# eladhoffer/convNet.pytorch

Measured on NVIDIA H100. Metric: ResNet-50 images/sec (training step, synthetic 224x224), higher is better.
Workload: dtype bf16

## Files before the change

### convnet/pytorch_b200/csrc/bn.cu

```cuda
#include "bn_common.cuh"

namespace b200 {

static inline int reduce_blocks(long long M, int C, const RowMap& rm, int resident_per_sm = 6) {
  long long iters = (M + rm.rows_per_iter - 1) / rm.rows_per_iter;
  long long want = (iters + 7) / 8;
  long long cap = 1200000LL / (2 * C);
  if (cap < sm_count()) cap = sm_count();
  if (cap > resident_per_sm * sm_count()) cap = resident_per_sm * sm_count();
  if (want > cap) want = cap;
  if (want < 1) want = 1;
  return (int)want;
}
__device__ __forceinline__ bool accumulate_and_elect(float (&acc)[16], int cv, int rows_per_iter, int C,
                                                     double* accum, unsigned* ticket) {
  __shared__ float red[kBnThreads][17];
  __shared__ bool is_last;
  const int t = threadIdx.x;
#pragma unroll
  for (int i = 0; i < 16; ++i) red[t][i] = acc[i];
  __syncthreads();
  for (int o = t; o < 2 * C; o += kBnThreads) {
    const int stat = o / C;
    const int c = o - stat * C;
// ... 348 lines not shown
    unsigned long long rm = 0;
    bool ok[ROWS];
    if (SRC == 2) rm = mask_rows<ROWS>(amask, r, C >> 3, (int)(col >> 3)) >> (col & 7 & ~(VEC - 1));
#pragma unroll
    for (int u = 0; u < ROWS; ++u) {
      const long long rr = r + (long long)u * rstep;
      ok[u] = rr < row_end;
      if (ok[u]) {
        rd[u] = ldv(dy + rr * C + col, (RawVec<VEC>*)nullptr);
        rz[u] = ldv(z + rr * C + col, (RawVec<VEC>*)nullptr);
        if (SRC == 1) ry[u] = ldv(y + rr * C + col, (RawVec<VEC>*)nullptr);
      }
    }
#pragma unroll
    for (int u = 0; u < ROWS; ++u) {
      if (!ok[u]) continue;
      const long long rr = r + (long long)u * rstep;
      float da[VEC], za[VEC], ya[VEC];
      unpackv(rd[u], da);
      unpackv(rz[u], za);
      if (SRC == 1) unpackv(ry[u], ya);
#pragma unroll
      for (int i = 0; i < VEC; ++i) {
        float g = da[i];
        if (SRC == 2) g = ((rm >> (8 * u + i)) & 1ull) ? g : 0.f;
        else if (act != B200_ACT_NONE && act_mask(SRC == 1 ? ya[i] : fmaf(za[i], A[i], sh[i]), act) == 0.f) g = 0.f;
        da[i] = g;
        za[i] = A[i] * g + B[i] * za[i] + Cc[i];
      }
      storev(dz + rr * C + col, za);
      if (g_out) storev(g_out + rr * C + col, da);
    }
  }
}

static inline double* ws_accum(float* ws) { return reinterpret_cast<double*>(ws); }
static inline unsigned* ws_ticket(float* ws) { return reinterpret_cast<unsigned*>(ws + kReplicas * 2 * kBnMaxC * 2); }

}

using namespace b200;

extern "C" size_t b200_bn_workspace_floats(int C) { (void)C; return (size_t)kWsFloats; }
extern "C" size_t b200_bn_act_mask_bytes(long long M, int C) { return (size_t)((M + 7) / 8 * 8) * (size_t)(C / 8); }

extern "C" int b200_bn_stats(const void* z, long long M, int C, const float* gamma, const float* beta, float eps,
                             float momentum, float* running_mean, float* running_var, long long* nbt, float* mean,
                             float* invstd, float* scale, float* shift, float* workspace, b200_stream_t stream_) {
  int rc = check_c(C, "bn_stats");
  if (rc) return rc;
  B200_REQUIRE(z && mean && invstd && scale && shift && workspace && M > 0, B200_ERR_INVALID, "bn_stats: bad argument");
  B200_REQUIRE((reinterpret_cast<uintptr_t>(workspace) & 7) == 0, B200_ERR_INVALID, "bn_stats: workspace misaligned");
  const RowMap rm = make_rowmap(C);
  b200::launch(bn_stats_kernel, reduce_blocks(M, C, rm), kBnThreads, 0, (cudaStream_t)stream_,
      (const __nv_bfloat16*)z, M, C, rm.cv, rm.rows_per_iter, gamma, beta, eps, momentum, running_mean, running_var,
      nbt, mean, invstd, scale, shift, ws_accum(workspace), ws_ticket(workspace));
  B200_CHECK_LAUNCH("bn_stats_kernel");
  return B200_OK;
}

extern "C" int b200_bn_finalize(long long M, int C, const float* gamma, const float* beta, float eps, float momentum,
                                float* running_mean, float* running_var, long long* nbt, float* mean, float* invstd,
                                float* scale, float* shift, float* workspace, b200_stream_t stream_) {
  int rc = check_c(C, "bn_finalize");
  if (rc) return rc;
  B200_REQUIRE(mean && invstd && scale && shift && workspace && M > 0, B200_ERR_INVALID, "bn_finalize: bad argument");
// ... 47 lines not shown
extern "C" int b200_bn_bwd_reduce(const void* dy, const void* y, const uint8_t* act_mask, const void* z, long long M,
                                  int C, int act,
                                  const float* mean, const float* invstd, const float* gamma, const float* beta,
                                  float* sums, float* dgamma_acc, float* dbeta_acc, float* workspace,
                                  b200_stream_t stream_) {
  int rc = check_c(C, "bn_bwd_reduce");
  if (rc) return rc;
  B200_REQUIRE(dy && z && mean && invstd && sums && workspace && M > 0, B200_ERR_INVALID, "bn_bwd_reduce: bad argument");
  const int src = (act == B200_ACT_NONE) ? 0 : (act_mask != nullptr ? 2 : (y != nullptr ? 1 : 0));
#define B200_RED_ARGS(VEC)                                                                                     \
  (const __nv_bfloat16*)dy, (const __nv_bfloat16*)y, act_mask, (const __nv_bfloat16*)z, M, C, rm.cv,           \
      rm.rows_per_iter, act, mean, invstd, gamma, beta, partial
#define B200_LAUNCH_RED(VEC, ROWS, MINB)                                                                       \
  do {                                                                                                         \
    const RowMap rm = make_rowmap_v<VEC>(C);                                                                   \
    blocks = partial_blocks(M, rm, MINB);                                                                      \
    if (src == 2)                                                                                              \
      b200::launch(bn_bwd_reduce_kernel<VEC, ROWS, MINB, 2>, blocks, kBnThreads, 0, stream, B200_RED_ARGS(VEC));         \
    else if (src == 1)                                                                                         \
      b200::launch(bn_bwd_reduce_kernel<VEC, ROWS, MINB, 1>, blocks, kBnThreads, 0, stream, B200_RED_ARGS(VEC));         \
    else                                                                                                       \
      b200::launch(bn_bwd_reduce_kernel<VEC, ROWS, MINB, 0>, blocks, kBnThreads, 0, stream, B200_RED_ARGS(VEC));         \
  } while (0)
  cudaStream_t stream = (cudaStream_t)stream_;
  float* partial = workspace + kAccumFloats;
  int blocks = 0;
  if (C > 1024)
    B200_LAUNCH_RED(8, 2, 3);
  else
    B200_LAUNCH_RED(4, 4, 4);
#undef B200_LAUNCH_RED
#undef B200_RED_ARGS
  B200_CHECK_LAUNCH("bn_bwd_reduce_kernel");
  b200::launch(bn_bwd_reduce_final_kernel, (2 * C + 3) / 4, kBnThreads, 0, stream, partial, blocks, C, sums, dgamma_acc,
                                                                           dbeta_acc);
  B200_CHECK_LAUNCH("bn_bwd_reduce_final_kernel");
  return B200_OK;
}

extern "C" int b200_bn_bwd_dx(const void* dy, const void* y, const uint8_t* act_mask, const void* z, long long M, int C,
                              int act,
                              const float* mean, const float* invstd, const float* gamma, const float* beta,
                              const float* sums, void* dz, void* g_out, b200_stream_t stream_) {
  int rc = check_c(C, "bn_bwd_dx");
  if (rc) return rc;
  B200_REQUIRE(dy && z && mean && invstd && sums && dz && M > 0, B200_ERR_INVALID, "bn_bwd_dx: bad argument");
  const int src = (act == B200_ACT_NONE) ? 0 : (act_mask != nullptr ? 2 : (y != nullptr ? 1 : 0));
#define B200_DX_ARGS(VEC)                                                                                    \
  (const __nv_bfloat16*)dy, (const __nv_bfloat16*)y, act_mask, (const __nv_bfloat16*)z, M, C, rm.cv,         \
      rm.rows_per_iter, act, mean, invstd, gamma, beta, sums, (__nv_bfloat16*)dz, (__nv_bfloat16*)g_out
#define B200_LAUNCH_DX(VEC, ROWS, MINB)                                                                      \
  do {                                                                                                       \
    const RowMap rm = make_rowmap_v<VEC>(C);                                                                 \
    const int blocks = stream_blocks(M, rm);                                                                 \
    if (src == 2)                                                                                            \
      b200::launch(bn_bwd_dx_kernel<VEC, ROWS, MINB, 2>, blocks, kBnThreads, 0, (cudaStream_t)stream_, B200_DX_ARGS(VEC)); \
    else if (src == 1)                                                                                       \
      b200::launch(bn_bwd_dx_kernel<VEC, ROWS, MINB, 1>, blocks, kBnThreads, 0, (cudaStream_t)stream_, B200_DX_ARGS(VEC)); \
    else                                                                                                     \
      b200::launch(bn_bwd_dx_kernel<VEC, ROWS, MINB, 0>, blocks, kBnThreads, 0, (cudaStream_t)stream_, B200_DX_ARGS(VEC)); \
  } while (0)
  if (C > 1024)
    B200_LAUNCH_DX(8, 2, 3);
  else
    B200_LAUNCH_DX(4, 4, 4);
#undef B200_LAUNCH_DX
#undef B200_DX_ARGS
  B200_CHECK_LAUNCH("bn_bwd_dx_kernel");
  return B200_OK;
}
// ... 1 lines not shown
```

### convnet/pytorch_b200/csrc/bn_common.cuh

```cuda
#pragma once
#include "common.cuh"
#include "host.h"

namespace b200 {

constexpr int kBnThreads = 256;
constexpr int kBnMaxC = 2048;
constexpr int kBnMaxBlocks = 1184;
constexpr int kAccumFloats = kReplicas * 2 * kBnMaxC * 2 + 64;
constexpr int kMaxPartialBlocks = 6 * 148;
constexpr int kWsFloats = kAccumFloats + kMaxPartialBlocks * 2 * kBnMaxC;

struct RowMap {
  int cv, rows_per_iter;
};
static inline RowMap make_rowmap(int C) {
  RowMap m;
  m.cv = C / 8;
  m.rows_per_iter = kBnThreads / m.cv;
  return m;
}
static inline int partial_blocks(long long M, const RowMap& rm, int resident_per_sm) {
  long long iters = (M + rm.rows_per_iter - 1) / rm.rows_per_iter;
  long long want = (iters + 3) / 4;
// ... 73 lines not shown
__device__ __forceinline__ RawVec<8> ldv(const __nv_bfloat16* p, RawVec<8>*) {
  RawVec<8> r;
  r.u = ld_stream(p);
  return r;
}
__device__ __forceinline__ void unpackv(const RawVec<4>& r, float (&f)[4]) {
  const float2 a = unpack_bf16x2(r.u.x), b = unpack_bf16x2(r.u.y);
  f[0] = a.x; f[1] = a.y; f[2] = b.x; f[3] = b.y;
}
__device__ __forceinline__ void unpackv(const RawVec<8>& r, float (&f)[8]) { unpack8(r.u, f); }
__device__ __forceinline__ void storev(__nv_bfloat16* p, const float (&f)[4]) {
  uint2 u;
  u.x = pack_bf16x2(f[0], f[1]); u.y = pack_bf16x2(f[2], f[3]);
  *reinterpret_cast<uint2*>(p) = u;
}
__device__ __forceinline__ void storev(__nv_bfloat16* p, const float (&f)[8]) { store8(p, f); }
template <int VEC>
__device__ __forceinline__ void loadfv(const float* p, float (&f)[VEC]) {
#pragma unroll
  for (int i = 0; i < VEC; i += 4) {
    const float4 a = __ldg(reinterpret_cast<const float4*>(p + i));
    f[i] = a.x; f[i + 1] = a.y; f[i + 2] = a.z; f[i + 3] = a.w;
  }
}

template <int VEC>
static inline RowMap make_rowmap_v(int C) {
  RowMap m;
  m.cv = C / VEC;
  m.rows_per_iter = kBnThreads / m.cv;
  return m;
}

static int check_c(int C, const char* who) {
  B200_REQUIRE(C > 0 && C % 8 == 0 && C <= kBnMaxC, B200_ERR_UNSUPPORTED,
               "%s: C=%d must be a multiple of 8 and <= %d", who, C, kBnMaxC);
  return B200_OK;
}

}
```

### convnet/pytorch_b200/engine.py

```python
import torch
import torch.nn as nn

from . import ops
from .lib import B200Error, ACT_NONE, ACT_RELU, ACT_RELU6

_ALIGN = 64
FOLD_BN_EVAL = True


def _round_up(n, m):
    return (n + m - 1) // m * m


class _Slot(object):
    __slots__ = ('name', 'param', 'kind', 'offset', 'numel', 'alloc', 'shape', 'group', 'module')


class Arena(object):

    def __init__(self, model, device):
        self.device = device
        self.convs = []
        self.version = 0
        self.grads_zero = False
# ... 369 lines not shown
                            m.num_batches_tracked, u.mean, u.invstd, u.scale, u.shift, self._ws)
        elif training:
            ops.bn_stats(u.z, bn.gamma, bn.beta, m.eps, m.momentum, m.running_mean, m.running_var,
                         m.num_batches_tracked, u.mean, u.invstd, u.scale, u.shift, self._ws)
        else:
            self._eval_coeffs(bn, u.scale, u.shift)
        bias = getattr(u.conv, 'bias32', None) if u.conv is not None else None
        if bias is not None:
            if training:
                if m.momentum is None:
                    m.running_mean.add_(bias / m.num_batches_tracked.to(torch.float32))
                else:
                    m.running_mean.add_(bias, alpha=float(m.momentum))
            else:
                u.shift.add_(u.scale * bias)

    def _stats_only(self, x, conv, bn, training):
        if not training and FOLD_BN_EVAL and not self._want_tape:
            return self._unit_fwd_folded(x, conv, bn, ACT_NONE)
        N, H, W, _ = x.shape
        u = _Unit()
        u.conv, u.bn, u.act, u.x = conv, bn, ACT_NONE, x
        u.desc = conv.desc(N, H, W)
        u.w = conv.kernel_weights()
        self._conv_and_coeffs(u, x, u.w, training)
        u.y = None
        return u

    def _sync_bn_sums(self, sums):
        import torch.distributed as dist
        dist.all_reduce(sums, group=self.sync_bn_group)
        sums.mul_(1.0 / self.sync_bn_world)

    def _bn_bwd(self, u, dy, y_mask, act, want_g=False):
        bn = u.bn
        mask = getattr(u, 'mask', None) if y_mask is not None else None
        ops.bn_bwd_reduce(dy, y_mask, u.z, act, u.mean, u.invstd, bn.gamma, bn.beta, u.sums, bn.dgamma, bn.dbeta,
                          self._ws, act_mask=mask)
        if self.sync_bn_world > 1:
            self._sync_bn_sums(u.sums)
        g = torch.empty_like(dy) if want_g else None
        if bn.l1:
            dz = ops.bn_l1_bwd_dx(dy, y_mask, u.z, act, u.mean, u.invstd, u.sign_sum, bn.gamma, bn.beta, u.sums,
                                  g_out=g, act_mask=mask)
        else:
            dz = ops.bn_bwd_dx(dy, y_mask, u.z, act, u.mean, u.invstd, bn.gamma, bn.beta, u.sums, g_out=g,
                               act_mask=mask)
        return dz, g

    def _wgrad_async(self, fn, *operands):
        if self._wg_stream is None:
            fn()
            return
        ev = torch.cuda.Event()
        ev.record()
        self._wg_stream.wait_event(ev)
        with torch.cuda.stream(self._wg_stream):
            fn()
        self._wg_keep.append(operands)

    def _wgrad_join(self):
        if self._wg_stream is not None and self._wg_keep:
            torch.cuda.current_stream().wait_stream(self._wg_stream)
            self._wg_keep = []

    def _buckets_begin(self):
        self._bucket_hi = self.arena.group_end[0] if self.grad_bucket_hook is not None else None

    def _bucket_point(self, lo, force=False):
# ... 279 lines not shown
            else:
                dws = torch.zeros((K, 9, 16), device=self.device, dtype=torch.float32)
                ops.conv_wgrad(u.x, dz, u.desc, dws)
                self.stem_g32.view(K, 9, Cin).add_(dws[:, :, :Cin])
        self._wgrad_async(stem_wgrad, u.x, dz)

    def _block_fwd(self, spec, x, training):
        convs, bns = spec['convs'], spec['bns']
        units = []
        h = x
        for i in range(len(convs) - 1):
            u = self._unit_fwd(h, convs[i], bns[i], ACT_RELU, training, True)
            units.append(u)
            h = u.y
        down, se_tape = None, None
        if spec.get('se') is not None:
            r = x
            if spec['down'] is not None:
                down = self._unit_fwd(x, spec['down'][0], spec['down'][1], ACT_NONE, training, True)
                r = down.y
            r, se_tape = spec['se'].fwd(r)
            last = self._unit_fwd(h, convs[-1], bns[-1], ACT_RELU, training, True, residual=r)
        elif spec['down'] is not None:
            down = self._stats_only(x, spec['down'][0], spec['down'][1], training)
            last = self._unit_fwd(h, convs[-1], bns[-1], ACT_RELU, training, True, other=down)
        else:
            last = self._unit_fwd(h, convs[-1], bns[-1], ACT_RELU, training, True, residual=x)
        units.append(last)
        return last.y, {'units': units, 'down': down, 'se': se_tape}

    def _block_bwd(self, spec, saved, dy):
        units, down = saved['units'], saved['down']
        last = units[-1]
        dz, g = self._bn_bwd(last, dy, last.y, ACT_RELU, want_g=True)
        if saved.get('se') is not None:
            g = spec['se'].bwd(self, saved['se'], g)
        if down is not None:
            dzd, _ = self._bn_bwd(down, g, None, ACT_NONE)
            skip = self._conv_bwd(down, dzd)
        else:
            skip = g
        d = self._conv_bwd(last, dz)
        for u in reversed(units[1:-1]):
            dz, _ = self._bn_bwd(u, d, None, ACT_RELU)
            d = self._conv_bwd(u, dz)
        u = units[0]
        dz, _ = self._bn_bwd(u, d, None, ACT_RELU)
        return self._conv_bwd(u, dz, residual=skip)

    def run_forward(self, x, training, want_tape, mix=None, aug=None):
        self._want_tape = want_tape
        if training:
            self.arena.version += 1
        h, stem = self._stem_fwd(x, training, mix, aug)
        saved = []
        for spec in self.blocks:
            h, s = self._block_fwd(spec, h, training)
            saved.append(s if want_tape else None)
        out, head = self._head_fwd(h, training, want_tape)
        tape = {'stem': stem, 'blocks': saved, 'head': head} if want_tape else None
        return out, tape

    def run_backward(self, tape, dlogits, dl_bf16=None):
        self._transpose_weights()
        self._buckets_begin()
        d = self._head_bwd(tape['head'], dlogits, dl_bf16)
        for spec, saved in zip(reversed(self.blocks), reversed(tape['blocks'])):
            d = self._block_bwd(spec, saved, d)
            convs = spec['convs'] + ([spec['down'][0]] if spec['down'] is not None else [])
            self._bucket_point(self._spec_lo(convs))
        self._stem_bwd(tape['stem'], d)
        self._wgrad_join()
        self._buckets_end()


class MobileNetRuntime(Runtime):

    def _build(self):
        m, a = self.model, self.arena
        f = m.features
        conv0 = f.conv0[0]
# ... 178 lines not shown
```

### convnet/pytorch_b200/lib.py

```python
import ctypes
import os
import threading

_HERE = os.path.dirname(os.path.abspath(__file__))
LIB_PATH = os.environ.get("B200_LIB_PATH") or os.path.join(_HERE, "libb200conv.so")

ACT_NONE, ACT_RELU, ACT_RELU6 = 0, 1, 2
MIX_NONE, MIX_MIXUP, MIX_CUTMIX = 0, 1, 2


class B200Error(RuntimeError):
    pass


class ConvDesc(ctypes.Structure):
    _fields_ = [(n, ctypes.c_int) for n in
                ("N", "H", "W", "C", "K", "R", "S", "stride", "pad_h", "pad_w", "P", "Q",
                 "x_pixel_stride", "x_row_stride", "x_image_stride", "window")]


class Epilogue(ctypes.Structure):
    _fields_ = [("bias", ctypes.c_void_p), ("residual", ctypes.c_void_p),
                ("act", ctypes.c_int), ("out_fp32", ctypes.c_int), ("bn_stats_workspace", ctypes.c_void_p)]


_vp, _i, _ll, _f, _sz = ctypes.c_void_p, ctypes.c_int, ctypes.c_longlong, ctypes.c_float, ctypes.c_size_t
_dp = ctypes.POINTER(ConvDesc)
_ep = ctypes.POINTER(Epilogue)

SIGNATURES = {
    "b200_conv_fprop": [_dp, _vp, _vp, _vp, _ep, _vp],
    "b200_conv_dgrad": [_dp, _vp, _vp, _vp, _vp, _vp],
    "b200_conv_wgrad": [_dp, _vp, _vp, _vp, _vp, _sz, _vp],
    "b200_conv_wgrad_workspace_bytes": [],
    "b200_dwconv_fprop": [_dp, _vp, _vp, _vp, _vp],
    "b200_dwconv_dgrad": [_dp, _vp, _vp, _vp, _vp],
    "b200_dwconv_wgrad": [_dp, _vp, _vp, _vp, _vp, _sz, _vp],
    "b200_bn_workspace_floats": [_i],
    "b200_bn_act_mask_bytes": [_ll, _i],
    "b200_bn_stats": [_vp, _ll, _i, _vp, _vp, _f, _f, _vp, _vp, _vp, _vp, _vp, _vp, _vp, _vp, _vp],
    "b200_bn_finalize": [_ll, _i, _vp, _vp, _f, _f, _vp, _vp, _vp, _vp, _vp, _vp, _vp, _vp, _vp],
    "b200_bn_eval_coeffs": [_i, _vp, _vp, _vp, _vp, _f, _vp, _vp, _vp],
    "b200_bn_apply": [_vp, _ll, _i, _vp, _vp, _vp, _vp, _vp, _vp, _i, _vp, _vp, _vp],
    "b200_bn_bwd_reduce": [_vp, _vp, _vp, _vp, _ll, _i, _i, _vp, _vp, _vp, _vp, _vp, _vp, _vp, _vp, _vp],
    "b200_bn_bwd_dx": [_vp, _vp, _vp, _vp, _ll, _i, _i, _vp, _vp, _vp, _vp, _vp, _vp, _vp, _vp],
    "b200_bn_l1_stats": [_vp, _ll, _i, _vp, _vp, _f, _f, _vp, _vp, _vp, _vp, _vp, _vp, _vp, _vp, _vp],
    "b200_bn_l1_eval_coeffs": [_i, _vp, _vp, _vp, _vp, _vp, _vp, _vp],
    "b200_bn_l1_bwd_dx": [_vp, _vp, _vp, _vp, _ll, _i, _i, _vp, _vp, _vp, _vp, _vp, _vp, _vp, _vp, _vp],
    "b200_maxpool3x3s2_fwd": [_vp, _i, _i, _i, _i, _vp, _vp, _vp],
    "b200_maxpool3x3s2_bwd": [_vp, _vp, _i, _i, _i, _i, _vp, _vp],
    "b200_bn_apply_maxpool3x3s2": [_vp, _i, _i, _i, _i, _vp, _vp, _i, _vp, _vp, _vp],
    "b200_avgpool_fwd": [_vp, _i, _i, _i, _vp, _vp],
    "b200_avgpool_bwd": [_vp, _i, _i, _i, _vp, _vp],
    "b200_input_prep": [_vp, _i, _i, _i, _i, _i, _i, _vp, _vp],
    "b200_input_prep_u8": [_vp, _i, _i, _i, _i, _i, _i, ctypes.POINTER(ctypes.c_float), ctypes.POINTER(ctypes.c_float),
                           _vp, _vp],
    "b200_input_prep_mix": [_vp, _i, _i, _i, _i, _i, _i, _vp, _vp, _i, _vp, _vp],
    "b200_input_prep_u8_mix": [_vp, _i, _i, _i, _i, _i, _i, ctypes.POINTER(ctypes.c_float),
                               ctypes.POINTER(ctypes.c_float), _vp, _vp, _i, _vp, _vp],
    "b200_input_prep_u8_aug": [_vp, _i, _i, _i, _i, _i, _i, _i, _vp, _vp, _i, _vp, _vp],
    "b200_input_prep_u8_rrc": [_vp, _ll, _vp, _vp, _i, _i, _i, _i, _i, _i, _i, _vp, _vp, _vp],
    "b200_weight_transpose": [_vp, _vp, _i, _i, _i, _vp],
    "b200_weight_transpose_batched": [_vp, _vp, _vp, _i, _i, _vp],
    "b200_stem_weight_to_s2d": [_vp, _i, _i, _i, _vp, _vp],
    "b200_stem_wgrad_from_s2d": [_vp, _i, _i, _i, _vp, _vp],
    "b200_cast_f32_to_bf16": [_vp, _vp, _ll, _vp],
    "b200_group_weight_pack": [_vp, _i, _i, _i, _i, _i, _i, _vp, _vp],
    "b200_group_wgrad_unpack": [_vp, _i, _i, _i, _i, _i, _vp, _vp],
    "b200_se_pool": [_vp, _i, _i, _i, _vp, _vp],
    "b200_se_scale_fwd": [_vp, _vp, _i, _i, _i, _vp, _vp],
    "b200_se_bwd_reduce": [_vp, _vp, _vp, _i, _i, _i, _vp, _vp],
    "b200_se_bwd_dx": [_vp, _vp, _vp, _i, _i, _i, _vp, _vp],
    "b200_act_bwd": [_vp, _vp, _ll, _i, _vp, _vp],
    "b200_softmax_ce": [_vp, _vp, _i, _i, _i, _f, _f, _vp, _vp, _vp, _vp, _vp],
    "b200_softmax_ce_mix": [_vp, _vp, _vp, _vp, _i, _i, _i, _f, _vp, _vp, _vp, _vp, _vp],
    "b200_colsum_bf16": [_vp, _i, _i, _vp, _vp],
    "b200_fused_sgd": [_vp, _vp, _vp, _vp, _ll, _ll, _f, _f, _f, _f, _f, _vp, _i, _i, _vp],
    "b200_sumsq": [_vp, _ll, _vp, _vp, _vp],
# ... 50 lines not shown
```

### convnet/pytorch_b200/ops.py

```python
import ctypes

import torch

from . import lib as _l
from .lib import ACT_NONE, ACT_RELU, ACT_RELU6, ConvDesc, Epilogue

bf16 = torch.bfloat16


def _stream():
    return torch.cuda.current_stream().cuda_stream


_TIMING = None


class _T(object):
    __slots__ = ('name', 'flops', 'nbytes', 'e0')

    def __init__(self, name, flops=0, nbytes=0):
        self.name, self.flops, self.nbytes = name, flops, nbytes

    def __enter__(self):
        if _TIMING is not None:
# ... 208 lines not shown
                 "b200_bn_bwd_reduce")


def bn_bwd_dx(dy, y, z, act, mean, invstd, gamma, beta, sums, dz=None, g_out=None, act_mask=None):
    C = z.shape[-1]
    M = z.numel() // C
    if dz is None:
        dz = torch.empty_like(z)
    with _T('bn_bwd_dx', 0, 2 * z.numel() * (3 + (y is not None and act_mask is None) + (g_out is not None))):
        _l.check(_l.load().b200_bn_bwd_dx(dy.data_ptr(), _l.ptr(y), _l.ptr(act_mask), z.data_ptr(), M, C, int(act),
                                          mean.data_ptr(),
                                          invstd.data_ptr(), _l.ptr(gamma), _l.ptr(beta), sums.data_ptr(),
                                          dz.data_ptr(), _l.ptr(g_out), _stream()), "b200_bn_bwd_dx")
    return dz


def bn_l1_stats(z, gamma, beta, eps, momentum, running_mean, running_var, mean, invstd, sign_sum, scale, shift,
                workspace):
    C = z.shape[-1]
    M = z.numel() // C
    _chk(z, bf16, "z")
    with _T('bn_l1_stats', 0, 2 * 2 * z.numel()):
        _l.check(_l.load().b200_bn_l1_stats(z.data_ptr(), M, C, _l.ptr(gamma), _l.ptr(beta), float(eps),
                                            float(momentum), _l.ptr(running_mean), _l.ptr(running_var),
                                            mean.data_ptr(), invstd.data_ptr(), sign_sum.data_ptr(), scale.data_ptr(),
                                            shift.data_ptr(), workspace.data_ptr(), _stream()), "b200_bn_l1_stats")


def bn_l1_eval_coeffs(gamma, beta, running_mean, running_var, scale, shift):
    C = running_mean.numel()
    _l.check(_l.load().b200_bn_l1_eval_coeffs(C, _l.ptr(gamma), _l.ptr(beta), running_mean.data_ptr(),
                                              running_var.data_ptr(), scale.data_ptr(), shift.data_ptr(), _stream()),
             "b200_bn_l1_eval_coeffs")


def bn_l1_bwd_dx(dy, y, z, act, mean, invstd, sign_sum, gamma, beta, sums, dz=None, g_out=None, act_mask=None):
    C = z.shape[-1]
    M = z.numel() // C
    _chk(dy, bf16, "dy"); _chk(y, bf16, "y"); _chk(z, bf16, "z"); _chk(act_mask, torch.uint8, "act_mask")
    if dz is None:
        dz = torch.empty_like(z)
    with _T('bn_l1_bwd_dx', 0, 2 * z.numel() * (3 + (y is not None and act_mask is None) + (g_out is not None))):
        _l.check(_l.load().b200_bn_l1_bwd_dx(dy.data_ptr(), _l.ptr(y), _l.ptr(act_mask), z.data_ptr(), M, C, int(act),
                                             mean.data_ptr(), invstd.data_ptr(), sign_sum.data_ptr(), _l.ptr(gamma),
                                             _l.ptr(beta), sums.data_ptr(), dz.data_ptr(), _l.ptr(g_out), _stream()),
                 "b200_bn_l1_bwd_dx")
    return dz


def _out(out, shape, dtype, device, name):
    if out is None:
        return torch.empty(shape, device=device, dtype=dtype)
    _chk(out, dtype, name)
    if tuple(out.shape) != tuple(shape):
        raise _l.B200Error("%s has shape %s, expected %s" % (name, tuple(out.shape), tuple(shape)))
    return out


def maxpool_fwd(x, want_argmax=True, out=None, argmax_out=None):
    N, H, W, C = x.shape
    OH, OW = (H - 1) // 2 + 1, (W - 1) // 2 + 1
    y = _out(out, (N, OH, OW, C), bf16, x.device, "out")
    am = _out(argmax_out, (N, OH, OW, C), torch.uint8, x.device, "argmax_out") if want_argmax else None
    with _T('maxpool_fwd', 0, 2 * x.numel() + 3 * y.numel()):
        _l.check(_l.load().b200_maxpool3x3s2_fwd(x.data_ptr(), N, H, W, C, y.data_ptr(), _l.ptr(am), _stream()),
                 "b200_maxpool3x3s2_fwd")
# ... 375 lines not shown
```

### include/b200conv.h

```cpp
#ifndef B200CONV_H_
#define B200CONV_H_

#include <stddef.h>
#include <stdint.h>

#ifdef __cplusplus
extern "C" {
#endif

typedef void* b200_stream_t;

#define B200_OK 0
#define B200_ERR_INVALID (-1)
#define B200_ERR_UNSUPPORTED (-2)
#define B200_ERR_CUDA (-3)

#define B200_ACT_NONE 0
#define B200_ACT_RELU 1
#define B200_ACT_RELU6 2

typedef struct {
  int N, H, W, C;
  int K, R, S;
  int stride;
// ... 19 lines not shown
                    const b200_epilogue* ep, b200_stream_t stream);
int b200_conv_dgrad(const b200_conv_desc* d, const void* dy, const void* wt, void* dx,
                    const void* residual, b200_stream_t stream);
size_t b200_conv_wgrad_workspace_bytes(void);
int b200_conv_wgrad(const b200_conv_desc* d, const void* x, const void* dy, float* dw,
                    void* workspace, size_t workspace_bytes, b200_stream_t stream);

int b200_dwconv_fprop(const b200_conv_desc* d, const void* x, const void* w, void* y, b200_stream_t stream);
int b200_dwconv_dgrad(const b200_conv_desc* d, const void* dy, const void* w, void* dx, b200_stream_t stream);
int b200_dwconv_wgrad(const b200_conv_desc* d, const void* x, const void* dy, float* dw,
                      float* workspace, size_t workspace_bytes, b200_stream_t stream);

size_t b200_bn_workspace_floats(int C);
int b200_bn_stats(const void* z, long long M, int C, const float* gamma, const float* beta,
                  float eps, float momentum, float* running_mean, float* running_var,
                  long long* num_batches_tracked, float* mean, float* invstd, float* scale, float* shift,
                  float* workspace, b200_stream_t stream);
int b200_bn_finalize(long long M, int C, const float* gamma, const float* beta, float eps, float momentum,
                     float* running_mean, float* running_var, long long* num_batches_tracked, float* mean,
                     float* invstd, float* scale, float* shift, float* workspace, b200_stream_t stream);
int b200_bn_eval_coeffs(int C, const float* gamma, const float* beta, const float* running_mean,
                        const float* running_var, float eps, float* scale, float* shift, b200_stream_t stream);
size_t b200_bn_act_mask_bytes(long long M, int C);
int b200_bn_apply(const void* z, long long M, int C, const float* scale, const float* shift,
                  const void* residual, const void* z2, const float* scale2, const float* shift2,
                  int act, void* y, uint8_t* act_mask, b200_stream_t stream);
int b200_bn_bwd_reduce(const void* dy, const void* y, const uint8_t* act_mask, const void* z, long long M, int C, int act,
                       const float* mean, const float* invstd, const float* gamma, const float* beta,
                       float* sums, float* dgamma_acc, float* dbeta_acc, float* workspace, b200_stream_t stream);
int b200_bn_bwd_dx(const void* dy, const void* y, const uint8_t* act_mask, const void* z, long long M, int C, int act,
                   const float* mean, const float* invstd, const float* gamma, const float* beta,
                   const float* sums, void* dz, void* g_out, b200_stream_t stream);

int b200_bn_l1_stats(const void* z, long long M, int C, const float* gamma, const float* beta, float eps,
                     float momentum, float* running_mean, float* running_var, float* mean, float* invstd,
                     float* sign_sum, float* scale, float* shift, float* workspace, b200_stream_t stream);
int b200_bn_l1_eval_coeffs(int C, const float* gamma, const float* beta, const float* running_mean,
                           const float* running_var, float* scale, float* shift, b200_stream_t stream);
int b200_bn_l1_bwd_dx(const void* dy, const void* y, const uint8_t* act_mask, const void* z, long long M, int C,
                      int act, const float* mean, const float* invstd, const float* sign_sum, const float* gamma,
                      const float* beta, const float* sums, void* dz, void* g_out, b200_stream_t stream);

int b200_maxpool3x3s2_fwd(const void* x, int N, int H, int W, int C, void* y, uint8_t* argmax, b200_stream_t stream);
int b200_maxpool3x3s2_bwd(const void* dy, const uint8_t* argmax, int N, int H, int W, int C, void* dx, b200_stream_t stream);
int b200_bn_apply_maxpool3x3s2(const void* z, int N, int H, int W, int C, const float* scale, const float* shift,
                               int act, void* y, uint8_t* argmax, b200_stream_t stream);
int b200_avgpool_fwd(const void* x, int N, int HW, int C, void* y, b200_stream_t stream);
int b200_avgpool_bwd(const void* dy, int N, int HW, int C, void* dx, b200_stream_t stream);

int b200_input_prep(const float* x_nchw, int N, int C, int H, int W, int Cpad, int mode, void* out, b200_stream_t stream);
int b200_input_prep_u8(const uint8_t* x_nhwc, int N, int C, int H, int W, int Cpad, int mode, const float* scale_host,
                       const float* bias_host, void* out, b200_stream_t stream);
#define B200_MIX_NONE 0
#define B200_MIX_MIXUP 1
#define B200_MIX_CUTMIX 2
typedef struct {
  float lam;
  int r0, r1, c0, c1;
} b200_mix_params;
int b200_input_prep_mix(const float* x_nchw, int N, int C, int H, int W, int Cpad, int mode, const long long* perm,
                        const b200_mix_params* params, int kind, void* out, b200_stream_t stream);
int b200_input_prep_u8_mix(const uint8_t* x_nhwc, int N, int C, int H, int W, int Cpad, int mode, const float* scale_host,
                           const float* bias_host, const long long* perm, const b200_mix_params* params, int kind,
                           void* out, b200_stream_t stream);
int b200_input_prep_u8_aug(const uint8_t* x_nhwc, int N, int D, int C, int H, int W, int Cpad, int pad, const float* lut,
                           const int16_t* params, int holes, void* out, b200_stream_t stream);
// ... 42 lines not shown
```

Measured before the change: 6590.

## Fuse last-BN and downsample-BN backward into joint reduce and dx kernels

In downsample bottleneck blocks without SE, the backward pass for the final BN and the downsample BN now runs through joint kernels. These read dy, the ReLU mask and both pre-BN activations once and produce both units' gradient statistics and both dz tensors. The intermediate gradient g is no longer written and re-read, and two reduce/dx kernel pairs become one pair. The cost is more registers per thread, and the two partial buffers now share one workspace, which limits how many blocks the reduce can use.

```diff
diff --git a/convnet/pytorch_b200/csrc/bn.cu b/convnet/pytorch_b200/csrc/bn.cu
--- a/convnet/pytorch_b200/csrc/bn.cu
+++ b/convnet/pytorch_b200/csrc/bn.cu
@@ -404,6 +404,14 @@
       if (g_out) storev(g_out + rr * C + col, da);
     }
   }
+}
+
+int launch_bn_bwd_reduce_final(const float* partial, int nblocks, int C, float* sums, float* dgamma_acc,
+                               float* dbeta_acc, cudaStream_t stream) {
+  b200::launch(bn_bwd_reduce_final_kernel, (2 * C + 3) / 4, kBnThreads, 0, stream, partial, nblocks, C, sums, dgamma_acc,
+               dbeta_acc);
+  B200_CHECK_LAUNCH("bn_bwd_reduce_final_kernel");
+  return B200_OK;
 }
 
 static inline double* ws_accum(float* ws) { return reinterpret_cast<double*>(ws); }
@@ -517,10 +525,7 @@
 #undef B200_LAUNCH_RED
 #undef B200_RED_ARGS
   B200_CHECK_LAUNCH("bn_bwd_reduce_kernel");
-  b200::launch(bn_bwd_reduce_final_kernel, (2 * C + 3) / 4, kBnThreads, 0, stream, partial, blocks, C, sums, dgamma_acc,
-                                                                           dbeta_acc);
-  B200_CHECK_LAUNCH("bn_bwd_reduce_final_kernel");
-  return B200_OK;
+  return launch_bn_bwd_reduce_final(partial, blocks, C, sums, dgamma_acc, dbeta_acc, stream);
 }
 
 extern "C" int b200_bn_bwd_dx(const void* dy, const void* y, const uint8_t* act_mask, const void* z, long long M, int C,
diff --git a/convnet/pytorch_b200/csrc/bn_common.cuh b/convnet/pytorch_b200/csrc/bn_common.cuh
--- a/convnet/pytorch_b200/csrc/bn_common.cuh
+++ b/convnet/pytorch_b200/csrc/bn_common.cuh
@@ -129,6 +129,9 @@
   return m;
 }
 
+int launch_bn_bwd_reduce_final(const float* partial, int nblocks, int C, float* sums, float* dgamma_acc,
+                               float* dbeta_acc, cudaStream_t stream);
+
 static int check_c(int C, const char* who) {
   B200_REQUIRE(C > 0 && C % 8 == 0 && C <= kBnMaxC, B200_ERR_UNSUPPORTED,
                "%s: C=%d must be a multiple of 8 and <= %d", who, C, kBnMaxC);
diff --git a/convnet/pytorch_b200/csrc/bn_join.cu b/convnet/pytorch_b200/csrc/bn_join.cu
--- /dev/null
+++ b/convnet/pytorch_b200/csrc/bn_join.cu
@@ -0,0 +1,221 @@
+#include "bn_common.cuh"
+
+namespace b200 {
+
+template <int VEC, int ROWS, int LB>
+__global__ void __launch_bounds__(kBnThreads, LB) bn_join_bwd_reduce_kernel(
+    const __nv_bfloat16* __restrict__ dy, const uint8_t* __restrict__ amask, const __nv_bfloat16* __restrict__ za,
+    const __nv_bfloat16* __restrict__ zb, long long M, int C, int cv, int rows_per_iter,
+    const float* __restrict__ mean_a, const float* __restrict__ invstd_a, const float* __restrict__ mean_b,
+    const float* __restrict__ invstd_b, float* __restrict__ partial_a, float* __restrict__ partial_b) {
+  const int t = threadIdx.x;
+  const bool active = t < rows_per_iter * cv;
+  const int r0 = t / cv, v = t - r0 * cv;
+  const long long rows_per_block = ((M + gridDim.x - 1) / gridDim.x + 7) & ~7LL;
+  const long long row_begin = blockIdx.x * rows_per_block;
+  const long long row_end = min(M, row_begin + rows_per_block);
+  float acc[3 * VEC];
+#pragma unroll
+  for (int i = 0; i < 3 * VEC; ++i) acc[i] = 0.f;
+  if (active) {
+    float mua[VEC], mub[VEC];
+    loadfv<VEC>(mean_a + v * VEC, mua);
+    loadfv<VEC>(mean_b + v * VEC, mub);
+    const long long col = (long long)v * VEC;
+    for (long long r = row_begin + (long long)r0 * ROWS; r < row_end; r += (long long)ROWS * rows_per_iter) {
+      RawVec<VEC> rd[ROWS], rza[ROWS], rzb[ROWS];
+      bool ok[ROWS];
+      const unsigned long long rm = mask_rows<ROWS>(amask, r, C >> 3, (int)(col >> 3)) >> (col & 7 & ~(VEC - 1));
+#pragma unroll
+      for (int u = 0; u < ROWS; ++u) {
+        const long long rr = r + u;
+        ok[u] = rr < row_end;
+        if (ok[u]) {
+          rd[u] = ldv(dy + rr * C + col, (RawVec<VEC>*)nullptr);
+          rza[u] = ldv(za + rr * C + col, (RawVec<VEC>*)nullptr);
+          rzb[u] = ldv(zb + rr * C + col, (RawVec<VEC>*)nullptr);
+        }
+      }
+#pragma unroll
+      for (int u = 0; u < ROWS; ++u) {
+        if (!ok[u]) continue;
+        float da[VEC], fa[VEC], fb[VEC];
+        unpackv(rd[u], da);
+        unpackv(rza[u], fa);
+        unpackv(rzb[u], fb);
+#pragma unroll
+        for (int i = 0; i < VEC; ++i) {
+          const float g = ((rm >> (8 * u + i)) & 1ull) ? da[i] : 0.f;
+          acc[i] = fmaf(g, fa[i] - mua[i], acc[i]);
+          acc[VEC + i] += g;
+          acc[2 * VEC + i] = fmaf(g, fb[i] - mub[i], acc[2 * VEC + i]);
+        }
+      }
+    }
+    float isa[VEC], isb[VEC];
+    loadfv<VEC>(invstd_a + v * VEC, isa);
+    loadfv<VEC>(invstd_b + v * VEC, isb);
+#pragma unroll
+    for (int i = 0; i < VEC; ++i) {
+      acc[i] *= isa[i];
+      acc[2 * VEC + i] *= isb[i];
+    }
+  }
+  __shared__ float red[kBnThreads][3 * VEC + 1];
+#pragma unroll
+  for (int i = 0; i < 3 * VEC; ++i) red[t][i] = acc[i];
+  __syncthreads();
+  float* dst_a = partial_a + (size_t)blockIdx.x * 2 * C;
+  float* dst_b = partial_b + (size_t)blockIdx.x * 2 * C;
+  for (int o = t; o < 2 * C; o += kBnThreads) {
+    const int stat = o / C;
+    const int c = o - stat * C;
+    const int vv = c / VEC, e = c - vv * VEC;
+    float sa = 0.f, sb = 0.f;
+    for (int r = 0; r < rows_per_iter; ++r) {
+      sa += red[r * cv + vv][stat * VEC + e];
+      sb += red[r * cv + vv][(2 - stat) * VEC + e];
+    }
+    dst_a[o] = sa;
+    dst_b[o] = sb;
+  }
+}
+
+template <int VEC, int ROWS, int LB>
+__global__ void __launch_bounds__(kBnThreads, LB) bn_join_bwd_dx_kernel(
+    const __nv_bfloat16* __restrict__ dy, const uint8_t* __restrict__ amask, const __nv_bfloat16* __restrict__ za,
+    const __nv_bfloat16* __restrict__ zb, long long M, int C, int cv, int rows_per_iter,
+    const float* __restrict__ mean_a, const float* __restrict__ invstd_a, const float* __restrict__ gamma_a,
+    const float* __restrict__ sums_a, const float* __restrict__ mean_b, const float* __restrict__ invstd_b,
+    const float* __restrict__ gamma_b, const float* __restrict__ sums_b, __nv_bfloat16* __restrict__ dza,
+    __nv_bfloat16* __restrict__ dzb) {
+  const int t = threadIdx.x;
+  if (t >= rows_per_iter * cv) return;
+  const int r0 = t / cv, v = t - r0 * cv;
+  const long long rows_per_block = ((M + gridDim.x - 1) / gridDim.x + 7) & ~7LL;
+  const long long row_begin = blockIdx.x * rows_per_block;
+  const long long row_end = min(M, row_begin + rows_per_block);
+  float Aa[VEC], Ba[VEC], Ca[VEC], Ab[VEC], Bb[VEC], Cb[VEC];
+  {
+    const float invM = 1.f / (float)M;
+    const float* mean[2] = {mean_a, mean_b};
+    const float* invstd[2] = {invstd_a, invstd_b};
+    const float* gamma[2] = {gamma_a, gamma_b};
+    const float* sums[2] = {sums_a, sums_b};
+#pragma unroll
+    for (int k = 0; k < 2; ++k) {
+      float mu[VEC], is[VEC], dg[VEC], dbt[VEC], A[VEC];
+      loadfv<VEC>(mean[k] + v * VEC, mu);
+      loadfv<VEC>(invstd[k] + v * VEC, is);
+      if (gamma[k]) loadfv<VEC>(gamma[k] + v * VEC, A);
+      loadfv<VEC>(sums[k] + v * VEC, dg);
+      loadfv<VEC>(sums[k] + C + v * VEC, dbt);
+#pragma unroll
+      for (int i = 0; i < VEC; ++i) {
+        const float gm = gamma[k] ? A[i] : 1.f;
+        const float a = gm * is[i];
+        const float b = -gm * is[i] * is[i] * dg[i] * invM;
+        const float cc = -a * dbt[i] * invM - b * mu[i];
+        if (k == 0) { Aa[i] = a; Ba[i] = b; Ca[i] = cc; } else { Ab[i] = a; Bb[i] = b; Cb[i] = cc; }
+      }
+    }
+  }
+  const long long col = (long long)v * VEC;
+  for (long long r = row_begin + (long long)r0 * ROWS; r < row_end; r += (long long)ROWS * rows_per_iter) {
+    RawVec<VEC> rd[ROWS], rza[ROWS], rzb[ROWS];
+    bool ok[ROWS];
+    const unsigned long long rm = mask_rows<ROWS>(amask, r, C >> 3, (int)(col >> 3)) >> (col & 7 & ~(VEC - 1));
+#pragma unroll
+    for (int u = 0; u < ROWS; ++u) {
+      const long long rr = r + u;
+      ok[u] = rr < row_end;
+      if (ok[u]) {
+        rd[u] = ldv(dy + rr * C + col, (RawVec<VEC>*)nullptr);
+        rza[u] = ldv(za + rr * C + col, (RawVec<VEC>*)nullptr);
+        rzb[u] = ldv(zb + rr * C + col, (RawVec<VEC>*)nullptr);
+      }
+    }
+#pragma unroll
+    for (int u = 0; u < ROWS; ++u) {
+      if (!ok[u]) continue;
+      const long long rr = r + u;
+      float da[VEC], fa[VEC], fb[VEC];
+      unpackv(rd[u], da);
+      unpackv(rza[u], fa);
+      unpackv(rzb[u], fb);
+#pragma unroll
+      for (int i = 0; i < VEC; ++i) {
+        const float g = ((rm >> (8 * u + i)) & 1ull) ? da[i] : 0.f;
+        fa[i] = Aa[i] * g + Ba[i] * fa[i] + Ca[i];
+        fb[i] = Ab[i] * g + Bb[i] * fb[i] + Cb[i];
+      }
+      storev(dza + rr * C + col, fa);
+      storev(dzb + rr * C + col, fb);
+    }
+  }
+}
+
+}
+
+using namespace b200;
+
+extern "C" int b200_bn_join_bwd_reduce(const void* dy, const uint8_t* act_mask, const void* z_a, const void* z_b,
+                                       long long M, int C, const float* mean_a, const float* invstd_a,
+                                       const float* mean_b, const float* invstd_b, float* sums_a, float* sums_b,
+                                       float* dgamma_a, float* dbeta_a, float* dgamma_b, float* dbeta_b,
+                                       float* workspace, b200_stream_t stream_) {
+  int rc = check_c(C, "bn_join_bwd_reduce");
+  if (rc) return rc;
+  B200_REQUIRE(dy && act_mask && z_a && z_b && mean_a && invstd_a && mean_b && invstd_b && sums_a && sums_b &&
+                   workspace && M > 0, B200_ERR_INVALID, "bn_join_bwd_reduce: bad argument");
+  cudaStream_t stream = (cudaStream_t)stream_;
+  float* partial_a = workspace + kAccumFloats;
+  int blocks = 0;
+  float* partial_b = nullptr;
+#define B200_LAUNCH_JRED(VEC, ROWS, MINB, LB)                                                                    \
+  do {                                                                                                           \
+    const RowMap rm = make_rowmap_v<VEC>(C);                                                                     \
+    blocks = partial_blocks(M, rm, MINB);                                                                        \
+    partial_b = partial_a + (size_t)blocks * 2 * C;                                                              \
+    B200_REQUIRE((size_t)blocks * 4 * C <= (size_t)kMaxPartialBlocks * 2 * kBnMaxC, B200_ERR_UNSUPPORTED,         \
+                 "bn_join_bwd_reduce: %d partial rows of two units exceed the workspace (C=%d)", blocks, C);      \
+    b200::launch(bn_join_bwd_reduce_kernel<VEC, ROWS, LB>, blocks, kBnThreads, 0, stream, (const __nv_bfloat16*)dy, \
+                 act_mask, (const __nv_bfloat16*)z_a, (const __nv_bfloat16*)z_b, M, C, rm.cv, rm.rows_per_iter,      \
+                 mean_a, invstd_a, mean_b, invstd_b, partial_a, partial_b);                                      \
+  } while (0)
+  if (C > 1024)
+    B200_LAUNCH_JRED(8, 2, 3, 2);
+  else
+    B200_LAUNCH_JRED(4, 4, 4, 3);
+#undef B200_LAUNCH_JRED
+  B200_CHECK_LAUNCH("bn_join_bwd_reduce_kernel");
+  rc = launch_bn_bwd_reduce_final(partial_a, blocks, C, sums_a, dgamma_a, dbeta_a, stream);
+  if (rc) return rc;
+  return launch_bn_bwd_reduce_final(partial_b, blocks, C, sums_b, dgamma_b, dbeta_b, stream);
+}
+
+extern "C" int b200_bn_join_bwd_dx(const void* dy, const uint8_t* act_mask, const void* z_a, const void* z_b,
+                                   long long M, int C, const float* mean_a, const float* invstd_a,
+                                   const float* gamma_a, const float* sums_a, const float* mean_b,
+                                   const float* invstd_b, const float* gamma_b, const float* sums_b, void* dz_a,
+                                   void* dz_b, b200_stream_t stream_) {
+  int rc = check_c(C, "bn_join_bwd_dx");
+  if (rc) return rc;
+  B200_REQUIRE(dy && act_mask && z_a && z_b && mean_a && invstd_a && sums_a && mean_b && invstd_b && sums_b && dz_a &&
+                   dz_b && M > 0, B200_ERR_INVALID, "bn_join_bwd_dx: bad argument");
+#define B200_LAUNCH_JDX(VEC, ROWS, LB)                                                                           \
+  do {                                                                                                           \
+    const RowMap rm = make_rowmap_v<VEC>(C);                                                                     \
+    b200::launch(bn_join_bwd_dx_kernel<VEC, ROWS, LB>, stream_blocks(M, rm), kBnThreads, 0, (cudaStream_t)stream_, \
+                 (const __nv_bfloat16*)dy, act_mask, (const __nv_bfloat16*)z_a, (const __nv_bfloat16*)z_b, M, C,     \
+                 rm.cv, rm.rows_per_iter, mean_a, invstd_a, gamma_a, sums_a, mean_b, invstd_b, gamma_b, sums_b,    \
+                 (__nv_bfloat16*)dz_a, (__nv_bfloat16*)dz_b);                                                      \
+  } while (0)
+  if (C > 1024)
+    B200_LAUNCH_JDX(8, 2, 2);
+  else
+    B200_LAUNCH_JDX(4, 4, 3);
+#undef B200_LAUNCH_JDX
+  B200_CHECK_LAUNCH("bn_join_bwd_dx_kernel");
+  return B200_OK;
+}
diff --git a/convnet/pytorch_b200/engine.py b/convnet/pytorch_b200/engine.py
--- a/convnet/pytorch_b200/engine.py
+++ b/convnet/pytorch_b200/engine.py
@@ -425,9 +425,9 @@
         dist.all_reduce(sums, group=self.sync_bn_group)
         sums.mul_(1.0 / self.sync_bn_world)
 
-    def _bn_bwd(self, u, dy, y_mask, act, want_g=False):
+    def _bn_bwd(self, u, dy, y_mask, act, want_g=False, act_mask=None):
         bn = u.bn
-        mask = getattr(u, 'mask', None) if y_mask is not None else None
+        mask = act_mask if act_mask is not None else (getattr(u, 'mask', None) if y_mask is not None else None)
         ops.bn_bwd_reduce(dy, y_mask, u.z, act, u.mean, u.invstd, bn.gamma, bn.beta, u.sums, bn.dgamma, bn.dbeta,
                           self._ws, act_mask=mask)
         if self.sync_bn_world > 1:
@@ -773,21 +773,44 @@
     def _block_bwd(self, spec, saved, dy):
         units, down = saved['units'], saved['down']
         last = units[-1]
-        dz, g = self._bn_bwd(last, dy, last.y, ACT_RELU, want_g=True)
-        if saved.get('se') is not None:
+        se = saved.get('se') is not None
+        ds_from_mask = down is not None and not se
+        if ds_from_mask and not last.bn.l1 and not down.bn.l1:
+            dz, dzd = self._bn_join_bwd(last, down, dy)
+            skip = self._conv_bwd(down, dzd)
+            d = self._conv_bwd(last, dz)
+            return self._block_bwd_rest(units, d, skip)
+        dz, g = self._bn_bwd(last, dy, last.y, ACT_RELU, want_g=not ds_from_mask)
+        if se:
             g = spec['se'].bwd(self, saved['se'], g)
-        if down is not None:
+        if ds_from_mask:
+            dzd, _ = self._bn_bwd(down, dy, last.y, ACT_RELU, act_mask=last.mask)
+            skip = self._conv_bwd(down, dzd)
+        elif down is not None:
             dzd, _ = self._bn_bwd(down, g, None, ACT_NONE)
             skip = self._conv_bwd(down, dzd)
         else:
             skip = g
         d = self._conv_bwd(last, dz)
+        return self._block_bwd_rest(units, d, skip)
+
+    def _block_bwd_rest(self, units, d, skip):
         for u in reversed(units[1:-1]):
             dz, _ = self._bn_bwd(u, d, None, ACT_RELU)
             d = self._conv_bwd(u, dz)
         u = units[0]
         dz, _ = self._bn_bwd(u, d, None, ACT_RELU)
         return self._conv_bwd(u, dz, residual=skip)
+
+    def _bn_join_bwd(self, last, down, dy):
+        a, b = last.bn, down.bn
+        ops.bn_join_bwd_reduce(dy, last.mask, last.z, down.z, last.mean, last.invstd, down.mean, down.invstd,
+                               last.sums, down.sums, a.dgamma, a.dbeta, b.dgamma, b.dbeta, self._ws)
+        if self.sync_bn_world > 1:
+            self._sync_bn_sums(last.sums)
+            self._sync_bn_sums(down.sums)
+        return ops.bn_join_bwd_dx(dy, last.mask, last.z, down.z, last.mean, last.invstd, a.gamma, last.sums,
+                                  down.mean, down.invstd, b.gamma, down.sums)
 
     def run_forward(self, x, training, want_tape, mix=None, aug=None):
         self._want_tape = want_tape
diff --git a/convnet/pytorch_b200/lib.py b/convnet/pytorch_b200/lib.py
--- a/convnet/pytorch_b200/lib.py
+++ b/convnet/pytorch_b200/lib.py
@@ -44,6 +44,9 @@
     "b200_bn_apply": [_vp, _ll, _i, _vp, _vp, _vp, _vp, _vp, _vp, _i, _vp, _vp, _vp],
     "b200_bn_bwd_reduce": [_vp, _vp, _vp, _vp, _ll, _i, _i, _vp, _vp, _vp, _vp, _vp, _vp, _vp, _vp, _vp],
     "b200_bn_bwd_dx": [_vp, _vp, _vp, _vp, _ll, _i, _i, _vp, _vp, _vp, _vp, _vp, _vp, _vp, _vp],
+    "b200_bn_join_bwd_reduce": [_vp, _vp, _vp, _vp, _ll, _i, _vp, _vp, _vp, _vp, _vp, _vp, _vp, _vp, _vp, _vp, _vp,
+                                _vp],
+    "b200_bn_join_bwd_dx": [_vp, _vp, _vp, _vp, _ll, _i, _vp, _vp, _vp, _vp, _vp, _vp, _vp, _vp, _vp, _vp, _vp],
     "b200_bn_l1_stats": [_vp, _ll, _i, _vp, _vp, _f, _f, _vp, _vp, _vp, _vp, _vp, _vp, _vp, _vp, _vp],
     "b200_bn_l1_eval_coeffs": [_i, _vp, _vp, _vp, _vp, _vp, _vp, _vp],
     "b200_bn_l1_bwd_dx": [_vp, _vp, _vp, _vp, _ll, _i, _i, _vp, _vp, _vp, _vp, _vp, _vp, _vp, _vp, _vp],
diff --git a/convnet/pytorch_b200/ops.py b/convnet/pytorch_b200/ops.py
--- a/convnet/pytorch_b200/ops.py
+++ b/convnet/pytorch_b200/ops.py
@@ -264,6 +264,38 @@
     _l.check(_l.load().b200_bn_l1_eval_coeffs(C, _l.ptr(gamma), _l.ptr(beta), running_mean.data_ptr(),
                                               running_var.data_ptr(), scale.data_ptr(), shift.data_ptr(), _stream()),
              "b200_bn_l1_eval_coeffs")
+
+
+def _chk_join(dy, act_mask, z_a, z_b):
+    _chk(dy, bf16, "dy"); _chk(z_a, bf16, "z_a"); _chk(z_b, bf16, "z_b"); _chk(act_mask, torch.uint8, "act_mask")
+    C = z_a.shape[-1]
+    M = z_a.numel() // C
+    if dy.shape != z_a.shape or z_b.shape != z_a.shape or act_mask is None or act_mask.numel() != bn_act_mask_bytes(M, C):
+        raise _l.B200Error("bn_join: dy, z_a, z_b must share one [.., C] shape and act_mask must be its mask")
+    return M, C
+
+
+def bn_join_bwd_reduce(dy, act_mask, z_a, z_b, mean_a, invstd_a, mean_b, invstd_b, sums_a, sums_b, dgamma_a, dbeta_a,
+                       dgamma_b, dbeta_b, workspace):
+    M, C = _chk_join(dy, act_mask, z_a, z_b)
+    with _T('bn_bwd_reduce', 0, 2 * z_a.numel() * 3):
+        _l.check(_l.load().b200_bn_join_bwd_reduce(dy.data_ptr(), act_mask.data_ptr(), z_a.data_ptr(), z_b.data_ptr(), M,
+                                                   C, mean_a.data_ptr(), invstd_a.data_ptr(), mean_b.data_ptr(),
+                                                   invstd_b.data_ptr(), sums_a.data_ptr(), sums_b.data_ptr(),
+                                                   _l.ptr(dgamma_a), _l.ptr(dbeta_a), _l.ptr(dgamma_b), _l.ptr(dbeta_b),
+                                                   workspace.data_ptr(), _stream()), "b200_bn_join_bwd_reduce")
+
+
+def bn_join_bwd_dx(dy, act_mask, z_a, z_b, mean_a, invstd_a, gamma_a, sums_a, mean_b, invstd_b, gamma_b, sums_b):
+    M, C = _chk_join(dy, act_mask, z_a, z_b)
+    dz_a, dz_b = torch.empty_like(z_a), torch.empty_like(z_b)
+    with _T('bn_bwd_dx', 0, 2 * z_a.numel() * 5):
+        _l.check(_l.load().b200_bn_join_bwd_dx(dy.data_ptr(), act_mask.data_ptr(), z_a.data_ptr(), z_b.data_ptr(), M, C,
+                                               mean_a.data_ptr(), invstd_a.data_ptr(), _l.ptr(gamma_a), sums_a.data_ptr(),
+                                               mean_b.data_ptr(), invstd_b.data_ptr(), _l.ptr(gamma_b),
+                                               sums_b.data_ptr(), dz_a.data_ptr(), dz_b.data_ptr(), _stream()),
+                 "b200_bn_join_bwd_dx")
+    return dz_a, dz_b
 
 
 def bn_l1_bwd_dx(dy, y, z, act, mean, invstd, sign_sum, gamma, beta, sums, dz=None, g_out=None, act_mask=None):
diff --git a/include/b200conv.h b/include/b200conv.h
--- a/include/b200conv.h
+++ b/include/b200conv.h
@@ -75,6 +75,15 @@
                    const float* mean, const float* invstd, const float* gamma, const float* beta,
                    const float* sums, void* dz, void* g_out, b200_stream_t stream);
 
+int b200_bn_join_bwd_reduce(const void* dy, const uint8_t* act_mask, const void* z_a, const void* z_b, long long M,
+                            int C, const float* mean_a, const float* invstd_a, const float* mean_b,
+                            const float* invstd_b, float* sums_a, float* sums_b, float* dgamma_a, float* dbeta_a,
+                            float* dgamma_b, float* dbeta_b, float* workspace, b200_stream_t stream);
+int b200_bn_join_bwd_dx(const void* dy, const uint8_t* act_mask, const void* z_a, const void* z_b, long long M, int C,
+                        const float* mean_a, const float* invstd_a, const float* gamma_a, const float* sums_a,
+                        const float* mean_b, const float* invstd_b, const float* gamma_b, const float* sums_b,
+                        void* dz_a, void* dz_b, b200_stream_t stream);
+
 int b200_bn_l1_stats(const void* z, long long M, int C, const float* gamma, const float* beta, float eps,
                      float momentum, float* running_mean, float* running_var, float* mean, float* invstd,
                      float* sign_sum, float* scale, float* shift, float* workspace, b200_stream_t stream);
```

After: 6728, median of 6. +2.1%, better.
